# daooshee/ReReVST-Code

Measured on AMD Instinct MI355X. Metric: stylized frames/sec at 512x512, 1 style, higher is better.
Workload: dtype f32

## Files before the change

### include/rerevst_hip.h

```cpp
#ifndef REREVST_HIP_H
#define REREVST_HIP_H

#include <stddef.h>
#include <stdint.h>

#ifdef __cplusplus
extern "C" {
#endif

typedef struct rrv_ctx* rrv_handle;

enum {
    RRV_OK = 0,
    RRV_E_ARG = -1,
    RRV_E_HIP = -2,
    RRV_E_WEIGHTS = -3,
    RRV_E_STATE = -4,
    RRV_E_NOMEM = -5,
    RRV_E_DEBUG = -6,
    RRV_E_COMM = -7
};

#define RRV_STATE_FLOATS 17536
#define RRV_MAX_STYLES 8
// ... 96 lines not shown
#define RRV_TF_ON_STREAM 4
int rrv_transfer_image_device(rrv_handle h, const void* d_in, rrv_image_desc in, int B, int H, int W,
                              void* d_out, rrv_image_desc out, int flags, void* hip_stream);

#define RRV_TF_WEIGHTS_DEVICE (1 << 3)
int rrv_transfer_image_blend_device(rrv_handle h, const void* d_in, rrv_image_desc in, int B, int H, int W,
                                    const float* style_weight, int n_styles,
                                    void* d_out, rrv_image_desc out, int flags, void* hip_stream);
int rrv_transfer_blend_batch(rrv_handle h, const uint8_t* frames_bgr, int B, int H, int W,
                             const float* style_weight, int n_styles, int pad_crop, float* out_bgr),
    rrv_transfer_blend_batch_u8(rrv_handle h, const uint8_t* frames_bgr, int B, int H, int W,
                                const float* style_weight, int n_styles, int pad_crop, uint8_t* out_bgr);

int rrv_transfer_image_mask_device(rrv_handle h, const void* d_in, rrv_image_desc in, int B, int H, int W,
                                   const float* d_mask, int n_styles, int mask_images,
                                   void* d_out, rrv_image_desc out, int flags, void* hip_stream);
int rrv_transfer_mask_batch(rrv_handle h, const uint8_t* frames_bgr, int B, int H, int W,
                            const float* mask, int n_styles, int mask_images, int pad_crop, float* out_bgr),
    rrv_transfer_mask_batch_u8(rrv_handle h, const uint8_t* frames_bgr, int B, int H, int W,
                               const float* mask, int n_styles, int mask_images, int pad_crop, uint8_t* out_bgr);

int rrv_prepare_style_image_device(rrv_handle h, const void* d_style, rrv_image_desc in, int Hs, int Ws, int style_id, void* hip_stream);
int rrv_add_image_device(rrv_handle h, const void* d_frame, rrv_image_desc in, int H, int W, void* hip_stream);

int rrv_get_preclamp(rrv_handle h, float* out, int H, int W);
int rrv_get_preclamp_image(rrv_handle h, float* out, int H, int W, int b);

int rrv_sync(rrv_handle h);

int rrv_set_pipeline(rrv_handle h, int n_slots);

int rrv_set_grid_share(rrv_handle h, int share);

int rrv_set_host_io(rrv_handle h, int mode);

int rrv_debug_copy_tensor(rrv_handle h, int slot, int index, int H, int W, float* host, size_t cap, size_t* floats);

int rrv_debug_copy_tensor_ex(rrv_handle h, int slot, int index, int image, int H, int W, float* host, size_t cap, size_t* floats,
                             int* layout, int* channels);

#define RRV_DBG_STATE_SET 0
#define RRV_DBG_STYLE_PRED 1
int rrv_debug_copy_state(rrv_handle h, int what, int slot, int image, float* out, int n);

int rrv_set_caller_stream(rrv_handle h, void* hip_stream, int enable);

int rrv_host_alloc(size_t bytes, void** out);
int rrv_host_free(void* p);
int rrv_host_register(void* p, size_t bytes);
int rrv_host_unregister(void* p);

int rrv_set_debug(rrv_handle h, int level);
int rrv_debug_selftest(rrv_handle h);
int rrv_debug_fail_alloc(rrv_handle h, int nth);

int rrv_profile_begin(rrv_handle h);
int rrv_profile_end(rrv_handle h);
int rrv_profile_count(rrv_handle h);
int rrv_profile_entry(rrv_handle h, int i, const char** name, float* ms, double* flops, double* bytes,
                      double* flops_executed);

#ifdef __cplusplus
}
#endif
#endif
```

### rerevst-code_amd/_lib.py

```python
import ctypes as C
import os

HERE = os.path.dirname(os.path.abspath(__file__))
LIB_PATH = os.environ.get("RRV_LIB_PATH") or os.path.join(HERE, "librerevst_hip.so")
STATE_FLOATS = 17536
MAX_STYLES = 8

_lib = None


class ImageDesc(C.Structure):
    _fields_ = [("dtype", C.c_int), ("layout", C.c_int), ("space", C.c_int)]


DT_U8, DT_F32 = 0, 1
LAY_HWC_BGR, LAY_CHW_RGB = 0, 1
SP_PIXEL, SP_UNIT, SP_NORM = 0, 1, 2
TF_PAD_CROP, TF_FRAME_MODE, TF_ON_STREAM, TF_WEIGHTS_DEVICE = 1, 2, 4, 8
DBG_STATE_SET, DBG_STYLE_PRED = 0, 1

SYMBOLS = {
    "rrv_create": (C.c_int, [C.c_int, C.POINTER(C.c_void_p)]),
    "rrv_destroy": (C.c_int, [C.c_void_p]),
    "rrv_last_error": (C.c_char_p, [C.c_void_p]),
# ... 13 lines not shown
    "rrv_broadcast_state": (C.c_int, [C.c_void_p, C.c_void_p, C.c_int, C.c_int, C.c_int]),
    "rrv_transfer": (C.c_int, [C.c_void_p, C.c_void_p, C.c_int, C.c_int, C.c_void_p]),
    "rrv_transfer_async": (C.c_int, [C.c_void_p, C.c_void_p, C.c_int, C.c_int, C.c_void_p, C.POINTER(C.c_long)]),
    "rrv_transfer_wait": (C.c_int, [C.c_void_p, C.c_long]),
    "rrv_transfer_device": (C.c_int, [C.c_void_p, C.c_void_p, C.c_int, C.c_int, C.c_void_p]),
    "rrv_transfer_batch_device": (C.c_int, [C.c_void_p, C.c_void_p, C.c_int, C.c_int, C.c_int, C.c_void_p]),
    "rrv_transfer_blend_device": (C.c_int, [C.c_void_p, C.c_void_p, C.c_int, C.c_int, C.POINTER(C.c_float), C.c_int, C.c_void_p]),
    "rrv_transfer_batch": (C.c_int, [C.c_void_p, C.c_void_p, C.c_int, C.c_int, C.c_int, C.c_void_p]),
    "rrv_transfer_blend": (C.c_int, [C.c_void_p, C.c_void_p, C.c_int, C.c_int, C.POINTER(C.c_float), C.c_int, C.c_void_p]),
    "rrv_transfer_frames_device": (C.c_int, [C.c_void_p, C.c_void_p, C.c_int, C.c_int, C.c_int, C.c_void_p]),
    "rrv_transfer_frames": (C.c_int, [C.c_void_p, C.c_void_p, C.c_int, C.c_int, C.c_int, C.c_void_p]),
    "rrv_generate_content_features": (C.c_int, [C.c_void_p, C.c_void_p, C.c_int, C.c_int, C.POINTER(C.c_int)]),
    "rrv_generate_content_features_batch": (C.c_int, [C.c_void_p, C.c_void_p, C.c_int, C.c_int, C.c_int, C.POINTER(C.c_int)]),
    "rrv_add_patch": (C.c_int, [C.c_void_p, C.c_int]),
    "rrv_transfer_features": (C.c_int, [C.c_void_p, C.c_int, C.POINTER(C.c_float), C.c_int, C.c_void_p]),
    "rrv_transfer_features_batch": (C.c_int, [C.c_void_p, C.POINTER(C.c_int), C.POINTER(C.c_float), C.c_int, C.c_int, C.c_void_p]),
    "rrv_release_features": (C.c_int, [C.c_void_p]),
    "rrv_set_multistyle_group": (C.c_int, [C.c_void_p, C.c_int]),
    "rrv_set_f43": (C.c_int, [C.c_void_p, C.c_int]),
    "rrv_set_feature_cache_cap": (C.c_int, [C.c_void_p, C.c_size_t]),
    "rrv_feature_cache_info": (C.c_int, [C.c_void_p, C.POINTER(C.c_int), C.POINTER(C.c_int), C.POINTER(C.c_size_t)]),
    "rrv_transfer_frame_mode": (C.c_int, [C.c_void_p, C.c_void_p, C.c_int, C.c_int, C.c_void_p]),
    "rrv_transfer_frame_mode_batch_device": (C.c_int, [C.c_void_p, C.c_void_p, C.c_int, C.c_int, C.c_int, C.c_void_p]),
    "rrv_transfer_frame_mode_batch": (C.c_int, [C.c_void_p, C.c_void_p, C.c_int, C.c_int, C.c_int, C.c_void_p]),
    "rrv_transfer_frame_mode_frames_device": (C.c_int, [C.c_void_p, C.c_void_p, C.c_int, C.c_int, C.c_int, C.c_void_p]),
    "rrv_transfer_frame_mode_frames": (C.c_int, [C.c_void_p, C.c_void_p, C.c_int, C.c_int, C.c_int, C.c_void_p]),
    "rrv_transfer_image_device": (C.c_int, [C.c_void_p, C.c_void_p, ImageDesc, C.c_int, C.c_int, C.c_int, C.c_void_p, ImageDesc,
                                            C.c_int, C.c_void_p]),
    "rrv_transfer_image_blend_device": (C.c_int, [C.c_void_p, C.c_void_p, ImageDesc, C.c_int, C.c_int, C.c_int, C.c_void_p, C.c_int,
                                                  C.c_void_p, ImageDesc, C.c_int, C.c_void_p]),
    "rrv_transfer_blend_batch": (C.c_int, [C.c_void_p, C.c_void_p, C.c_int, C.c_int, C.c_int, C.POINTER(C.c_float), C.c_int, C.c_int, C.c_void_p]),
    "rrv_transfer_image_mask_device": (C.c_int, [C.c_void_p, C.c_void_p, ImageDesc, C.c_int, C.c_int, C.c_int, C.c_void_p, C.c_int, C.c_int,
                                                 C.c_void_p, ImageDesc, C.c_int, C.c_void_p]),
    "rrv_transfer_mask_batch": (C.c_int, [C.c_void_p, C.c_void_p, C.c_int, C.c_int, C.c_int, C.POINTER(C.c_float), C.c_int, C.c_int, C.c_int, C.c_void_p]),
    "rrv_prepare_style_image_device": (C.c_int, [C.c_void_p, C.c_void_p, ImageDesc, C.c_int, C.c_int, C.c_int, C.c_void_p]),
    "rrv_add_image_device": (C.c_int, [C.c_void_p, C.c_void_p, ImageDesc, C.c_int, C.c_int, C.c_void_p]),
    "rrv_get_preclamp": (C.c_int, [C.c_void_p, C.c_void_p, C.c_int, C.c_int]),
    "rrv_get_preclamp_image": (C.c_int, [C.c_void_p, C.c_void_p, C.c_int, C.c_int, C.c_int]),
    "rrv_sync": (C.c_int, [C.c_void_p]),
    "rrv_set_pipeline": (C.c_int, [C.c_void_p, C.c_int]),
    "rrv_set_host_io": (C.c_int, [C.c_void_p, C.c_int]),
    "rrv_debug_copy_tensor": (C.c_int, [C.c_void_p, C.c_int, C.c_int, C.c_int, C.c_int, C.c_void_p, C.c_size_t, C.POINTER(C.c_size_t)]),
    "rrv_debug_copy_tensor_ex": (C.c_int, [C.c_void_p, C.c_int, C.c_int, C.c_int, C.c_int, C.c_int, C.c_void_p, C.c_size_t,
                                           C.POINTER(C.c_size_t), C.POINTER(C.c_int), C.POINTER(C.c_int)]),
    "rrv_debug_copy_state": (C.c_int, [C.c_void_p, C.c_int, C.c_int, C.c_int, C.c_void_p, C.c_int]),
    "rrv_set_grid_share": (C.c_int, [C.c_void_p, C.c_int]),
    "rrv_set_caller_stream": (C.c_int, [C.c_void_p, C.c_void_p, C.c_int]),
    "rrv_host_alloc": (C.c_int, [C.c_size_t, C.POINTER(C.c_void_p)]),
    "rrv_host_free": (C.c_int, [C.c_void_p]),
    "rrv_host_register": (C.c_int, [C.c_void_p, C.c_size_t]),
    "rrv_host_unregister": (C.c_int, [C.c_void_p]),
    "rrv_set_debug": (C.c_int, [C.c_void_p, C.c_int]),
    "rrv_debug_selftest": (C.c_int, [C.c_void_p]),
    "rrv_debug_fail_alloc": (C.c_int, [C.c_void_p, C.c_int]),
    "rrv_profile_begin": (C.c_int, [C.c_void_p]),
    "rrv_profile_end": (C.c_int, [C.c_void_p]),
    "rrv_profile_count": (C.c_int, [C.c_void_p]),
    "rrv_profile_entry": (C.c_int, [C.c_void_p, C.c_int, C.POINTER(C.c_char_p), C.POINTER(C.c_float),
                                    C.POINTER(C.c_double), C.POINTER(C.c_double), C.POINTER(C.c_double)]),
}

U8_TWINS = ("rrv_transfer", "rrv_transfer_async", "rrv_transfer_batch", "rrv_transfer_frames", "rrv_transfer_device",
            "rrv_transfer_batch_device", "rrv_transfer_frames_device", "rrv_transfer_blend", "rrv_transfer_blend_device",
            "rrv_transfer_features", "rrv_transfer_features_batch", "rrv_transfer_frame_mode", "rrv_transfer_frame_mode_batch",
            "rrv_transfer_frame_mode_batch_device", "rrv_transfer_frame_mode_frames", "rrv_transfer_frame_mode_frames_device",
            "rrv_transfer_blend_batch", "rrv_transfer_mask_batch")
SYMBOLS.update({name + "_u8": SYMBOLS[name] for name in U8_TWINS})


def _share_torch_hip_runtime():
    if os.environ.get("RRV_SYSTEM_HIP") == "1":
        return
    try:
        import importlib.util
        spec = importlib.util.find_spec("torch")
        if spec and spec.submodule_search_locations:
            libdir = os.path.join(list(spec.submodule_search_locations)[0], "lib")
            cand = os.path.join(libdir, "libamdhip64.so")
            if os.path.exists(cand):
                C.CDLL(cand, mode=C.RTLD_GLOBAL)
            rccl = os.path.join(libdir, "librccl.so")
            if os.path.exists(rccl):
                os.environ.setdefault("RRV_RCCL_PATH", rccl)
    except Exception:
        pass


def load():
    global _lib
    if _lib is not None:
        return _lib
    if not os.path.exists(LIB_PATH):
        raise OSError("%s not found: build it with `python __graft_entry__.py build` "
                      "(hipcc --offload-arch=gfx950); there is no CPU fallback" % LIB_PATH)
    _share_torch_hip_runtime()
    lib = C.CDLL(LIB_PATH)
    for name, (res, args) in SYMBOLS.items():
        fn = getattr(lib, name)
        fn.restype, fn.argtypes = res, args
    _lib = lib
    return lib
```

### rerevst-code_amd/csrc/conv_ups5.h

```cpp
#pragma once

struct Ups5Tab {
    static constexpr int G2[5][3] = {{2, 0, 0}, {1, 1, 1}, {-1, -1, 1}, {-1, 1, 1}, {0, 0, 2}};
    static constexpr int BT4[4][4] = {{1, 0, -1, 0}, {0, 1, 1, 0}, {0, -1, 1, 0}, {0, -1, 0, 1}};
    static constexpr int AT[4][5] = {{1, 1, 0, -1, 0}, {0, 1, 1, 0, 0}, {0, 1, 0, 1, 0}, {0, 1, -1, 0, 1}};
    static constexpr int DS[5] = {0, 1, 2, 2, 3};
};
template <int T, int R>
constexpr int ups5_coef(int k) { return T == 0 ? Ups5Tab::BT4[R][k] : Ups5Tab::AT[R][k]; }
template <int T, int R, int N>
__device__ __forceinline__ f32x4 ups5_comb(const f32x4 (&x)[N]) {
    constexpr int F = [] { for (int k = 0; k < N; ++k) if (ups5_coef<T, R>(k) == 1) return k; return -1; }();
    static_assert(F >= 0, "every row has a +1 coefficient");
    f32x4 r = x[F];
    static_for([&](auto kc) {
        constexpr int k = decltype(kc)::value;
        constexpr int c = ups5_coef<T, R>(k);
        static_assert(c == 0 || c == 1 || c == -1, "0 / +-1 coefficients");
        if constexpr (k != F && c == 1) r = e4add(r, x[k]);
        else if constexpr (c == -1) r = f4sub(r, x[k]);
    }, std::make_integer_sequence<int, N>{});
    return r;
}

struct Ups5Geo {
    static constexpr int NT = 256, NB = 2;
    static constexpr int NPOS = 29;
    static constexpr int NUB = 26;
    static constexpr int NPIECE = 16;
    static constexpr int HALO = 18, HALF = 18 * 9;
    static constexpr int PIECES = HALO * HALO * 4;
    static constexpr int RAW_IT = (PIECES + NT - 1) / NT;
    static constexpr int RAW_BYTES = RAW_IT * NT * 16;
    static constexpr int U_BYTES = NUB * 32 * 16 * 4;
    static constexpr int U_IT = U_BYTES / 16 / NT;
    static_assert(U_IT * NT * 16 == U_BYTES, "U image is a whole number of LDS-DMA rounds");
    static constexpr int SMEM = 2 * RAW_BYTES + 2 * U_BYTES + WINO_PAR_BYTES;
    static_assert(SMEM <= 160 * 1024, "LDS");
    static constexpr int OCC = 1;
    static constexpr int vidx(int i) { return i < 25 ? Ups5Tab::DS[i % 5] * 4 + Ups5Tab::DS[i / 5] : (i == 25 ? 5 : i == 26 ? 9 : i == 27 ? 6 : 10); }
    static constexpr int issued(int j) { return (j + 2 < NUB ? 2 : 0) + (j < NPIECE ? 1 : 0); }
    static constexpr int younger(int i) {
        return i == 0 ? 2 + issued(0) : i == 1 ? issued(0) + issued(1) : (i - 2 < NPIECE ? 1 : 0) + issued(i - 1) + issued(i);
    }
    static constexpr int col_iter(int dx) { return 4 * dx + 6; }
    static constexpr int row_iter(int r) { return col_iter(3) + 1 + r; }
};
static_assert(Ups5Geo::row_iter(3) < Ups5Geo::NPOS, "next chunk transformed inside the MFMA loop");

template <int EPI, int PERIMG>
__device__ __forceinline__ void conv_ups5_body(const ConvP& p) {
    static_assert(!(EPI & (E_POOL | E_RES | E_RES_UPS | E_NORM2)), "conv1 epilogues only: bias, activation, saved-stat normalise");
    using G = Ups5Geo;
    constexpr int RAW_BYTES = G::RAW_BYTES, U_BYTES = G::U_BYTES, NT = G::NT, NB = G::NB, NPOS = G::NPOS, NUB = G::NUB;
    extern __shared__ __attribute__((aligned(16))) char smem[];
    const int tid = threadIdx.x;
    const int wave = __builtin_amdgcn_readfirstlane(tid >> 6);
    const int lane = tid & 63, t = lane & 15, q = lane >> 4;
    const int tr = t >> 3, tc = t & 7;
    const int tg = wave;
    const int nchunks = p.Cin >> 4;
    const int n_ntiles = p.Cout >> 5;

    struct Item { int tx, ty, b, nt; };
    Item cur, nxt, dlt;
    {
        const int GD = gridDim.x, w = blockIdx.x;
        int pix, dpix;
        if (p.xcd_slabs) {
            const int PT = (GD >> 3) / n_ntiles;
            pix = (w & 7) * PT + (w >> 3) / n_ntiles; dpix = 8 * PT;
            cur.nt = (w >> 3) % n_ntiles; dlt.nt = 0;
        } else {
            cur.nt = w % n_ntiles; pix = w / n_ntiles;
            dlt.nt = GD % n_ntiles; dpix = GD / n_ntiles;
        }
        cur.tx = pix % p.tiles_x; cur.ty = (pix / p.tiles_x) % p.tiles_y; cur.b = pix / (p.tiles_x * p.tiles_y);
        dlt.tx = dpix % p.tiles_x; dlt.ty = (dpix / p.tiles_x) % p.tiles_y; dlt.b = dpix / (p.tiles_x * p.tiles_y);
    }
    auto advance = [&](const Item& a) {
        Item r = a;
        r.nt += dlt.nt;
        int carry = 0;
        if (r.nt >= n_ntiles) { r.nt -= n_ntiles; carry = 1; }
        r.tx += dlt.tx + carry;
        if (r.tx >= p.tiles_x) { r.tx -= p.tiles_x; r.ty += 1; }
        r.ty += dlt.ty;
        if (r.ty >= p.tiles_y) { r.ty -= p.tiles_y; r.b += 1; }
        r.b += dlt.b;
        return r;
    };
    auto in_of = [&](const Item& a) {
        return p.in + (size_t)a.b * (size_t)(p.Hi + 2) * (p.Wi + 2) * p.Cin + (size_t)(((a.ty + p.ty0) * 16) * (p.Wi + 2) + (a.tx + p.tx0) * 16) * p.Cin;
    };
    auto w_of = [&](const Item& a) { return p.wpk + (size_t)a.nt * nchunks * (NUB * 32 * 16); };
    int asrc[G::RAW_IT];
#pragma unroll
    for (int it = 0; it < G::RAW_IT; ++it) {
        const int e = it * NT + tid;
        int P = e >> 2;
        const int qq = e & 3;
        if (P >= G::HALO * G::HALO) P = 0;
        const int hf = P >= G::HALF, rem = P - hf * G::HALF;
        const int hy = rem / 9, hx = 2 * (rem - hy * 9) + hf;
        asrc[it] = ((hy * (p.Wi + 2) + hx) * p.Cin + 4 * (qq ^ ((hx >> 1) & 3))) * 4;
    }
    const int raw_last_num = ((G::RAW_IT - 1) * NT + wave * 64 < G::PIECES) ? 0x7fffffff : 0;
    bool have = cur.b < p.B, have_nxt = false;
    const float* in_t = in_of(cur);
    const float* w_t = w_of(cur);
    const float* in_n = in_t;
    const float* w_n = w_t;
    auto stage_u = [&](int chunk) {
        char* udst = smem + 2 * RAW_BYTES + (chunk & 1) * U_BYTES;
#pragma unroll
        for (int it = 0; it < G::U_IT; ++it) bufld16(w_t, udst + (it * NT + wave * 64) * 16, tid * 16, chunk * U_BYTES + it * NT * 16);
    };
    auto stage_raw = [&](int chunk) {
        char* rdst = smem + (chunk & 1) * RAW_BYTES;
#pragma unroll
        for (int it = 0; it < G::RAW_IT; ++it)
            if (it * NT + wave * 64 < G::PIECES) bufld16(in_t, rdst + (it * NT + wave * 64) * 16, asrc[it], chunk * 64);
    };
    char* const par = smem + 2 * RAW_BYTES + 2 * U_BYTES;
    auto stage_params = [&](int ntile, int img) {
        if (wave < 2) {
            const int e = tid;
            const int row = e >> 3, col = (e & 7) * 4;
            const float* src = p.bias;
            const int pb = PERIMG ? img * p.par_bstride : 0;
            int off = ntile * 32 + col;
            if (row >= 1 && row <= 4) { src = (EPI & E_NORM1) ? p.n1 : p.bias; off = (EPI & E_NORM1) ? ntile * 32 + col + pb + (row - 1) * p.Cout : off; }
            if (row > 4) { src = p.bias; off = ntile * 32; }
            glds16(src + off, par + wave * 1024);
        }
    };

    const unsigned lds0 = (unsigned)(size_t)(__attribute__((address_space(3))) char*)smem;
    unsigned offD[4];
#pragma unroll
    for (int dx = 0; dx < 4; ++dx) {
        const int hy = 4 * tg + 2 * tr, hx = 2 * tc + dx;
        const int P = (hx & 1) * G::HALF + hy * 9 + (hx >> 1);
        offD[dx] = lds0 + P * 64 + ((q ^ ((hx >> 1) & 3)) << 4);
    }
    const unsigned offU = lds0 + 2 * RAW_BYTES + t * 64 + ((q ^ ((0 - (t >> 2)) & 3)) << 4);
    const unsigned offU1 = offU + U_BYTES;

    f32x4 acc[NPOS][NB];
    f32x4 va[16], vb[16];
    auto pass = [](f32x4& x0, f32x4& x1, f32x4& x2, f32x4& x3) {
        const f32x4 a[4] = {x0, x1, x2, x3};
        x0 = ups5_comb<0, 0>(a); x1 = ups5_comb<0, 1>(a); x2 = ups5_comb<0, 2>(a); x3 = ups5_comb<0, 3>(a);
    };
    auto col_pass = [&](f32x4 (&d)[16], int dx) { pass(d[dx * 4 + 0], d[dx * 4 + 1], d[dx * 4 + 2], d[dx * 4 + 3]); };
    auto row_pass = [&](f32x4 (&d)[16], int r) { pass(d[0 * 4 + r], d[1 * 4 + r], d[2 * 4 + r], d[3 * 4 + r]); };

    auto chunk_body = [&](int c, auto par_c, auto first_c, f32x4 (&vcur)[16], f32x4 (&vnext)[16]) {
        constexpr int PAR = decltype(par_c)::value;
        constexpr bool FIRST = decltype(first_c)::value;
        const bool own_u = c + 1 < nchunks, own_r = c + 2 < nchunks;
        const rsrc_t rs_u = make_rsrc(own_u ? w_t : w_n);
        const rsrc_t rs_r = make_rsrc(own_r ? in_t : in_n);
        const rsrc_t rs_rl = make_rsrc(own_r ? in_t : in_n, raw_last_num);
        const int usoff = own_u ? (c + 1) * U_BYTES : 0;
        const int rsoff = (own_r ? c + 2 : c + 2 - nchunks) * 64;
        char* const udst = smem + 2 * RAW_BYTES + (1 - PAR) * U_BYTES;
        char* const rdst = smem + PAR * RAW_BYTES;
        const unsigned ub = PAR ? offU1 : offU;
        constexpr int RB = (1 - PAR) * RAW_BYTES;
        f32x4 u[4][NB];
        f32x4 (&d)[16] = vnext;
        u[0][0] = lds_rd128<0>(ub);
        u[0][1] = lds_rd128<1024>(ub);
        u[1][0] = lds_rd128<2048>(ub);
        u[1][1] = lds_rd128<2048 + 1024>(ub);
        static_for([&](auto ic) {
            constexpr int i = decltype(ic)::value;
            if constexpr (i + 2 < NUB) {
                u[(i + 2) & 3][0] = lds_rd128<(i + 2) * 2048>(ub);
                u[(i + 2) & 3][1] = lds_rd128<(i + 2) * 2048 + 1024>(ub);
            }
            if constexpr (i < 16) d[i] = lds_rd128<RB + (i & 3) * 576>(offD[i >> 2]);
            constexpr int US = (i < NUB ? i : NUB - 1) & 3;
            if constexpr (i < NUB) {
                constexpr int cdx = (i - 6) / 4;
                if constexpr (i >= 6 && (i - 6) % 4 == 0 && cdx < 4) {
                    static_assert(G::col_iter(cdx) == i, "column release schedule");
                    asm volatile("s_waitcnt lgkmcnt(%6)" : "+v"(d[cdx * 4 + 0]), "+v"(d[cdx * 4 + 1]), "+v"(d[cdx * 4 + 2]), "+v"(d[cdx * 4 + 3]),
                                 "+v"(u[US][0]), "+v"(u[US][1]) : "i"(G::younger(i)));
                } else {
                    lds_release2<G::younger(i)>(u[US][0], u[US][1]);
                }
            }
            __builtin_amdgcn_sched_barrier(0);
            if constexpr (i < G::U_IT) bufld16_rs(rs_u, udst + (i * NT + wave * 64) * 16, tid * 16, usoff + i * NT * 16);
            if constexpr (i < G::RAW_IT) bufld16_rs(i == G::RAW_IT - 1 ? rs_rl : rs_r, rdst + (i * NT + wave * 64) * 16, asrc[i], rsoff);
            const f32x4 vv = vcur[G::vidx(i)];
#pragma unroll
            for (int s = 0; s < 4; ++s)
#pragma unroll
                for (int nb = 0; nb < NB; ++nb)
                    acc[i][nb] = __builtin_amdgcn_mfma_f32_16x16x4f32(u[US][nb][s], vv[s], (FIRST && s == 0) ? f32x4{0.f, 0.f, 0.f, 0.f} : acc[i][nb], 0, 0, 0);
            static_for([&](auto xc) {
                constexpr int k = decltype(xc)::value;
                if constexpr (G::col_iter(k) == i) col_pass(d, k);
                if constexpr (G::row_iter(k) == i) row_pass(d, k);
            }, std::make_integer_sequence<int, 4>{});
        }, std::make_integer_sequence<int, NPOS>{});
    };

    int par_ntile = -1, par_img = -1;
    if (have) {
        stage_raw(0);
        stage_u(0);
        stage_raw(1);
        stage_params(cur.nt, cur.b);
        par_ntile = cur.nt; par_img = cur.b;
        __syncthreads();
#pragma unroll
        for (int k = 0; k < 16; ++k) va[k] = *(const f32x4*)(smem + (offD[k >> 2] - lds0) + (k & 3) * 576);
#pragma unroll
        for (int dx = 0; dx < 4; ++dx) col_pass(va, dx);
#pragma unroll
        for (int r = 0; r < 4; ++r) row_pass(va, r);
        __syncthreads();
    }
    while (have) {
        const int e_y0 = (cur.ty + p.ty0) * 32, e_x0 = (cur.tx + p.tx0) * 32, e_b = cur.b, e_ntile = cur.nt;
        nxt = advance(cur);
        have_nxt = nxt.b < p.B;
        in_n = have_nxt ? in_of(nxt) : in_t;
        w_n = have_nxt ? w_of(nxt) : w_t;
        if (par_ntile != e_ntile || (PERIMG && par_img != e_b)) {
            __syncthreads();
            stage_params(e_ntile, e_b);
            par_ntile = e_ntile; par_img = e_b;
        }
        chunk_body(0, std::integral_constant<int, 0>{}, std::true_type{}, va, vb);
        __syncthreads();
        chunk_body(1, std::integral_constant<int, 1>{}, std::false_type{}, vb, va);
        __syncthreads();
        for (int c = 2; c < nchunks; c += 2) {
            chunk_body(c, std::integral_constant<int, 0>{}, std::false_type{}, va, vb);
            __syncthreads();
            chunk_body(c + 1, std::integral_constant<int, 1>{}, std::false_type{}, vb, va);
            __syncthreads();
        }
        cur = nxt; have = have_nxt; in_t = in_n; w_t = w_n;

        float* out_b = p.out + (size_t)e_b * (size_t)(p.H + 2) * (p.W + 2 + (p.out_p8 ? 6 : 0)) * p.Cout;
        const int yb = e_y0 + 8 * tg + 4 * tr, xb = e_x0 + 4 * tc;
        {
            const int ly0 = yb >> 1, lx0 = xb >> 1;
            float* sc_b = p.sc_out + (size_t)e_b * (size_t)(p.Hi + 2) * (p.Wi + 2) * p.Cout;
#pragma unroll
            for (int nb = 0; nb < NB; ++nb) {
                const f32x4 s0 = f4sub(acc[25][nb], acc[27][nb]), s1 = e4add(acc[25][nb], acc[27][nb]);
                const f32x4 t0 = f4sub(acc[26][nb], acc[28][nb]), t1 = e4add(acc[26][nb], acc[28][nb]);
                const f32x4 sc[2][2] = {{f4sub(s0, t0), e4add(s0, t0)}, {f4sub(s1, t1), e4add(s1, t1)}};
#pragma unroll
                for (int a = 0; a < 2; ++a)
#pragma unroll
                    for (int b = 0; b < 2; ++b) {
                        const int ly = ly0 + a, lx = lx0 + b;
                        if (ly < p.Hi && lx < p.Wi)
                            *(f32x4*)(sc_b + ((size_t)(ly + 1) * (p.Wi + 2) + lx + 1) * p.Cout + e_ntile * 32 + nb * 16 + 4 * q) = sc[a][b];
                    }
            }
        }
#pragma unroll
        for (int nb = 0; nb < NB; ++nb) {
            const int co = e_ntile * 32 + nb * 16 + 4 * q;
            f32x4 T[5][4];
#pragma unroll
            for (int r = 0; r < 5; ++r) {
                const f32x4 m[5] = {acc[r * 5 + 0][nb], acc[r * 5 + 1][nb], acc[r * 5 + 2][nb], acc[r * 5 + 3][nb], acc[r * 5 + 4][nb]};
                T[r][0] = ups5_comb<1, 0>(m); T[r][1] = ups5_comb<1, 1>(m); T[r][2] = ups5_comb<1, 2>(m); T[r][3] = ups5_comb<1, 3>(m);
            }
            f32x4 Y[4][4];
#pragma unroll
            for (int j = 0; j < 4; ++j) {
                const f32x4 tj[5] = {T[0][j], T[1][j], T[2][j], T[3][j], T[4][j]};
                Y[0][j] = ups5_comb<1, 0>(tj); Y[1][j] = ups5_comb<1, 1>(tj); Y[2][j] = ups5_comb<1, 2>(tj); Y[3][j] = ups5_comb<1, 3>(tj);
            }
            const char* pl = par + (nb * 16 + 4 * q) * 4;
            const f32x4 bias = *(const f32x4*)(pl);
            f32x4 m1, r1, lo1, hi1;
            if (EPI & E_NORM1) {
                m1 = *(const f32x4*)(pl + 128); r1 = *(const f32x4*)(pl + 256);
                lo1 = *(const f32x4*)(pl + 384); hi1 = *(const f32x4*)(pl + 512);
            }
#pragma unroll
            for (int i = 0; i < 4; ++i)
#pragma unroll
                for (int j = 0; j < 4; ++j) {
                    const int y = yb + i, x = xb + j;
                    f32x4 o = e4add(Y[i][j], bias);
                    if (EPI & E_RELU) o = f4relu(o);
                    if (EPI & E_LRELU) o = f4lrelu(o);
                    if (EPI & E_NORM1) o = f4norm_clamp(o, m1, r1, lo1, hi1);
                    if (y < p.H && x < p.W) {
                        if (p.out_p8) *(f32x4*)(out_b + (size_t)(co >> 3) * ((size_t)(p.H + 2) * (p.W + 8) * 8) + ((size_t)(y + 1) * (p.W + 8) + x + 4) * 8 + (co & 7)) = o;
                        else *(f32x4*)(out_b + ((size_t)(y + 1) * (p.W + 2) + x + 1) * p.Cout + co) = o;
                    }
                }
        }
    }
    asm volatile("s_waitcnt vmcnt(0)" ::: "memory");
}

__global__ void pack_ups5_k(const float* __restrict__ w, const float* __restrict__ wsc, float* __restrict__ dst, int Cout, int Cin) {
    constexpr int CH = 16, NUB = Ups5Geo::NUB;
    const size_t total = (size_t)Cout * Cin * NUB;
    for (size_t i = blockIdx.x * (size_t)blockDim.x + threadIdx.x; i < total; i += (size_t)gridDim.x * blockDim.x) {
        size_t r = i;
        const int cl = (int)(r % CH); r /= CH;
        const int j = r & 31; r >>= 5;
        const int pos = (int)(r % NUB); r /= NUB;
        const int nchunks = Cin / CH;
        const int chunk = r % nchunks; r /= nchunks;
        const int n_tile = (int)r;
        const int e = cl & 3, qs = cl >> 2;
        const int qq = qs ^ ((0 - (j >> 2)) & 3);
        const int co = n_tile * 32 + j, ci = chunk * CH + qq * 4 + e;
        if (pos == 25) { dst[i] = wsc[(size_t)co * Cin + ci] * 0.25f; continue; }
        const float* g = w + ((size_t)co * Cin + ci) * 9;
        auto G5 = [](int row, double g0, double g1, double g2) {
            return 0.5 * (Ups5Tab::G2[row][0] * g0 + Ups5Tab::G2[row][1] * g1 + Ups5Tab::G2[row][2] * g2);
        };
        const int pr = pos / 5, pc = pos % 5;
        double rowv[3];
#pragma unroll
        for (int kx = 0; kx < 3; ++kx) rowv[kx] = G5(pr, g[0 * 3 + kx], g[1 * 3 + kx], g[2 * 3 + kx]);
        dst[i] = (float)G5(pc, rowv[0], rowv[1], rowv[2]);
    }
}
```

### rerevst-code_amd/csrc/rerevst_hip.hip

```cpp
#include <hip/hip_runtime.h>
#include <dlfcn.h>
#include <stddef.h>
#include <stdint.h>
#include <string.h>
#include <algorithm>
#include <cmath>
#include <thread>
#include <stdio.h>
#include <map>
#include <condition_variable>
#include <mutex>
#include <string>
#include <vector>

#include "../../include/rerevst_hip.h"
#include "conv_mfma.h"
#include "conv_wino.h"
#include "conv_wino_split.h"
#include "conv_f43.h"
#include "conv_thin.h"
#include "prep_kernels.h"
#include "mask_kernels.h"

namespace {
// ... 1553 lines not shown
    if (const char* e = getenv("RRV_DEBUG")) h->debug = atoi(e) < 0 ? 0 : (atoi(e) > 2 ? 2 : atoi(e));
    *out = h;
    return RRV_OK;
}

static void free_plans(rrv_handle h) {
    for (auto& pair : h->enc_frame) for (EncPlan& e : pair) enc_free(e);
    enc_free(h->enc_add); enc_free(h->enc_style);
    for (auto& pair : h->dec) for (DecPlan& d : pair) dec_free(h, d);
    prep_free(h);
}

int rrv_set_debug(rrv_handle h, int level) {
    if (!h || level < 0 || level > 2) return RRV_E_ARG;
    HIPCHK(hipSetDevice(h->dev));
    RCHK(sync_all(h));
    free_plans(h);
    h->debug = level;
    return RRV_OK;
}

int rrv_debug_fail_alloc(rrv_handle h, int nth) {
    if (!h || nth < 0) return RRV_E_ARG;
    h->fail_alloc_in = nth;
    return RRV_OK;
}

__global__ void dbg_poke_k(float* p, long off) { p[off] = 1.0f; }
int rrv_debug_selftest(rrv_handle h) {
    if (!h) return RRV_E_ARG;
    HIPCHK(hipSetDevice(h->dev));
    RCHK(sync_all(h));
    const int saved = h->debug;
    h->debug = 2;
    Tens t;
    int rc = talloc(h, &t, 2, 8, 8, 64);
    if (rc == RRV_OK) rc = debug_verify(h, "selftest (clean)");
    int caught = 0;
    if (rc == RRV_OK) {
        hipLaunchKernelGGL(dbg_poke_k, dim3(1), dim3(1), 0, h->stream, t.p, (long)t.img_floats() + 5);
        if (debug_verify(h, "selftest (ring)") == RRV_E_DEBUG) ++caught;
        HIPCHK(hipMemsetAsync(t.p + t.img_floats(), 0, 64 * sizeof(float), h->stream));
        hipLaunchKernelGGL(dbg_poke_k, dim3(1), dim3(1), 0, h->stream, t.p, -3L);
        if (debug_verify(h, "selftest (guard)") == RRV_E_DEBUG) ++caught;
    }
    tfree(&t);
    h->debug = saved;
    if (rc != RRV_OK) return rc;
    if (caught != 2) return fail(h, RRV_E_DEBUG, "debug selftest: a deliberate out-of-bounds store was not detected");
    h->err.clear();
    return RRV_OK;
}

int rrv_destroy(rrv_handle h) {
    if (!h) return RRV_E_ARG;
    (void)hipSetDevice(h->dev);
    (void)hipDeviceSynchronize();
    for (auto& kv : h->conv) {
        if (kv.second.raw) (void)hipFree(kv.second.raw);
        if (kv.second.pk) (void)hipFree(kv.second.pk);
        if (kv.second.pk_ups) (void)hipFree(kv.second.pk_ups);
        if (kv.second.pk_ups_sc) (void)hipFree(kv.second.pk_ups_sc);
        if (kv.second.pk_wino) (void)hipFree(kv.second.pk_wino);
        if (kv.second.pk_f43) (void)hipFree(kv.second.pk_f43);
        if (kv.second.bias && kv.second.bias != h->zero_bias) (void)hipFree(kv.second.bias);
    }
    if (h->zero_bias) (void)hipFree(h->zero_bias);
    for (int f = 0; f < 3; ++f) {
        const ConvW &fd = h->sets[0].fold_down[f], &fu = h->sets[0].fold_up[f];
        for (float* q : {fd.raw, fd.bias, fd.pk_wino, fu.raw, fu.pk_wino}) if (q) (void)hipFree(q);
    }
    if (h->sets[0].active) (void)hipFree(h->sets[0].active);
    for (int i = 0; i < 6; ++i) { if (h->fc_w[i]) (void)hipFree(h->fc_w[i]); if (h->fc_b[i]) (void)hipFree(h->fc_b[i]); }
    if (h->fold_tmp) (void)hipFree(h->fold_tmp);
    for (float* p : h->patches) (void)hipFree(p);
    for (auto& f : h->features) if (f.owned) { if (f.p) (void)hipFree(f.p); if (f.u8) (void)hipFree(f.u8); }
    for (void* b : h->feat_blocks) (void)hipFree(b);
    free_plans(h);
    for (StyleState& s : h->styles) { if (s.blob) (void)hipFree(s.blob); if (s.smean) (void)hipFree(s.smean); tfree(&s.map); }
    if (h->d_u8) (void)hipFree(h->d_u8);
    if (h->d_outf) (void)hipFree(h->d_outf);
    if (h->pend_u8) (void)hipFree(h->pend_u8);
    for (auto& bw : h->blend_w) {
        if (bw.dev) (void)hipFree(bw.dev);
        if (bw.pin) (void)hipHostFree(bw.pin);
        for (hipEvent_t e : bw.ev) if (e) (void)hipEventDestroy(e);
    }
    if (h->stat_part) (void)hipFree(h->stat_part);
    for (float* q : {h->first_w[0], h->first_w[1], h->first_b[0], h->first_b[1], h->first_wg}) if (q) (void)hipFree(q);
    for (auto& st : h->hstage) {
        stage_free(st.pin, true);
        stage_free(st.dev, false);
        if (st.mask) (void)hipFree(st.mask);
        if (st.mask_pin) (void)hipHostFree(st.mask_pin);
        for (hipEvent_t e : {st.in_done, st.k_done, st.out_done}) if (e) (void)hipEventDestroy(e);
    }
    if (h->copy_in) (void)hipStreamDestroy(h->copy_in);
    if (h->copy_out) (void)hipStreamDestroy(h->copy_out);
    for (ProfEntry& e : h->prof) { (void)hipEventDestroy(e.e0); (void)hipEventDestroy(e.e1); }
    for (int i = 0; i < RRV_MAX_SLOTS; ++i) { (void)hipStreamDestroy(h->streams[i]); if (h->slot_ev[i]) (void)hipEventDestroy(h->slot_ev[i]); }
    delete h;
    return RRV_OK;
}

const char* rrv_last_error(rrv_handle h) { return h ? h->err.c_str() : "null handle"; }

// ... 1540 lines not shown
```

### rerevst-code_amd/framework.py

```python
import collections
import ctypes as C

import numpy as np

from . import _lib
from .weights import weight_table, load_checkpoint


class RRVError(RuntimeError):
    pass


def pinned_empty(shape, dtype=np.float32):
    import weakref
    lib = _lib.load()
    dt = np.dtype(dtype)
    n = int(np.prod(shape)) * dt.itemsize
    ptr = C.c_void_p()
    if lib.rrv_host_alloc(max(n, 1), C.byref(ptr)) != 0:
        raise MemoryError("rrv_host_alloc(%d) failed" % n)
    buf = (C.c_char * max(n, 1)).from_address(ptr.value)
    weakref.finalize(buf, lib.rrv_host_free, ptr)
    return np.frombuffer(buf, dtype=dt, count=int(np.prod(shape))).reshape(shape)

# ... 218 lines not shown
        self._h = C.c_void_p()
        rc = self._lib.rrv_create(self.device, C.byref(self._h))
        if rc != 0:
            self._h = None
            raise RRVError("rrv_create(device=%d) failed with %d (no HIP device?)" % (self.device, rc))
        weights = checkpoint if isinstance(checkpoint, dict) else load_checkpoint(checkpoint)
        for key, shape in weight_table().items():
            if key not in weights:
                raise KeyError("missing weight %s" % key)
            w = np.ascontiguousarray(weights[key], dtype=np.float32)
            if tuple(w.shape) != tuple(shape):
                raise ValueError("weight %s has shape %s, expected %s" % (key, w.shape, shape))
            shp = (C.c_int64 * w.ndim)(*w.shape)
            self._chk(self._lib.rrv_load_weight(self._h, key.encode(), w.ctypes.data_as(C.c_void_p), shp, w.ndim))
        self._chk(self._lib.rrv_finalize_weights(self._h))

    def _chk(self, rc):
        if rc != 0:
            msg = self._lib.rrv_last_error(self._h)
            err = RRVError("librerevst_hip error %d: %s" % (rc, msg.decode() if msg else "?"))
            err.code = rc
            raise err

    def close(self):
        if getattr(self, "_h", None):
            self._lib.rrv_destroy(self._h)
            self._h = None
        self._open = {}

    def __del__(self):
        try:
            self.close()
        except Exception:
            pass

    def _global_only(self, what):
        if not self.use_Global:
            raise RRVError("%s() belongs to Sequence-Level Global Feature Sharing (use_Global=True)" % what)

    def add(self, patch):
        self._global_only("add")
        a = _u8_image(patch, "patch")
        self._chk(self._lib.rrv_add(self._h, a.ctypes.data_as(C.c_void_p), a.shape[0], a.shape[1]))

    def compute(self):
        self._global_only("compute")
        self._chk(self._lib.rrv_compute(self._h))

    def set_debug(self, level):
        self._chk(self._lib.rrv_set_debug(self._h, int(level)))

    def debug_selftest(self):
        self._chk(self._lib.rrv_debug_selftest(self._h))

    def debug_fail_alloc(self, nth):
        self._chk(self._lib.rrv_debug_fail_alloc(self._h, int(nth)))

    def set_workspace_cap(self, nbytes):
        self._chk(self._lib.rrv_set_workspace_cap(self._h, int(nbytes)))

    def last_compute_info(self):
        g, n, b = C.c_int(), C.c_int(), C.c_size_t()
        self._chk(self._lib.rrv_last_compute_info(self._h, C.byref(g), C.byref(n), C.byref(b)))
        return g.value, n.value, b.value

    def clean(self):
        self._global_only("clean")
        self._chk(self._lib.rrv_clean(self._h))

    def prepare_style(self, style):
        styles = style if isinstance(style, (list, tuple)) else [style]
        for sid, s in enumerate(styles):
            a = _u8_image(s, "style")
            self._chk(self._lib.rrv_prepare_style(self._h, a.ctypes.data_as(C.c_void_p), a.shape[0], a.shape[1], sid))

    def _device_image(self, x, space, layout):
        import torch
        a = tensor_io_args(x, self.device, space=space, layout=layout)
        return a, C.c_void_p(torch.cuda.current_stream(x.device).cuda_stream)

    def prepare_style_tensor(self, style, *, space="pixel", layout="nchw"):
        styles = style if isinstance(style, (list, tuple)) else [style]
        for sid, s in enumerate(styles):
            a, stream = self._device_image(s, space, layout)
            if a.batched:
                raise ValueError("a style is one image: [3,H,W] or [H,W,3], got shape %s" % (tuple(s.shape),))
            self._chk(self._lib.rrv_prepare_style_image_device(self._h, C.c_void_p(a.x.data_ptr()), a.in_desc, a.H, a.W, sid, stream))

    def add_tensor(self, x, *, space="pixel", layout="nchw"):
        self._global_only("add")
        a, stream = self._device_image(x, space, layout)
        xb = a.x if a.batched else a.x.unsqueeze(0)
        for b in range(a.B):
            self._chk(self._lib.rrv_add_image_device(self._h, C.c_void_p(xb[b].data_ptr()), a.in_desc, a.H, a.W, stream))

    def transfer(self, frame, style_weight=None, dtype=np.float32):
        a = _u8_image(frame, "frame")
        H, W = a.shape[:2]
        out, u8 = _output((H // 8 * 8, W // 8 * 8, 3), dtype, None)
        if not self.use_Global:
            fn = self._lib.rrv_transfer_frame_mode_u8 if u8 else self._lib.rrv_transfer_frame_mode
            self._chk(fn(self._h, a.ctypes.data_as(C.c_void_p), H, W, out.ctypes.data_as(C.c_void_p)))
            return out
        if style_weight is None:
            fn = self._lib.rrv_transfer_u8 if u8 else self._lib.rrv_transfer
            rc = fn(self._h, a.__array_interface__["data"][0], H, W, out.__array_interface__["data"][0])
# ... 285 lines not shown
```

Before: 852.6.

## Spread ups5 conv prefetch requests across MFMA loop and double-buffer epilogue params

Spreads the global-to-LDS buffer loads for the next chunk's raw input and transformed weights evenly across the MFMA iterations (SPAN=25), where before they were issued in a burst at the first iterations. Epilogue parameters (bias and normalisation stats) are double-buffered in LDS and staged for the next tile during the current one, which removes an extra __syncthreads before each parameter restage. Adds compile-time ablation switches and a debug entry point for testing the conv kernel in isolation. The risk is different instruction scheduling and register pressure inside the hot loop.

```diff
diff --git a/include/rerevst_hip.h b/include/rerevst_hip.h
--- a/include/rerevst_hip.h
+++ b/include/rerevst_hip.h
@@ -172,6 +172,8 @@
 
 int rrv_set_debug(rrv_handle h, int level);
 int rrv_debug_selftest(rrv_handle h);
+int rrv_debug_conv_ups5(rrv_handle h, const float* in_ring, int B, int Hi, int Wi, int Cin, int Cout, const float* w, const float* wsc,
+                        const float* bias, const float* n1, int per_image, int out_p8, int grid_wgs, float* out, float* sc_out);
 int rrv_debug_fail_alloc(rrv_handle h, int nth);
 
 int rrv_profile_begin(rrv_handle h);
diff --git a/rerevst-code_amd/_lib.py b/rerevst-code_amd/_lib.py
--- a/rerevst-code_amd/_lib.py
+++ b/rerevst-code_amd/_lib.py
@@ -89,6 +89,8 @@
     "rrv_host_unregister": (C.c_int, [C.c_void_p]),
     "rrv_set_debug": (C.c_int, [C.c_void_p, C.c_int]),
     "rrv_debug_selftest": (C.c_int, [C.c_void_p]),
+    "rrv_debug_conv_ups5": (C.c_int, [C.c_void_p, C.c_void_p, C.c_int, C.c_int, C.c_int, C.c_int, C.c_int, C.c_void_p, C.c_void_p,
+                                      C.c_void_p, C.c_void_p, C.c_int, C.c_int, C.c_int, C.c_void_p, C.c_void_p]),
     "rrv_debug_fail_alloc": (C.c_int, [C.c_void_p, C.c_int]),
     "rrv_profile_begin": (C.c_int, [C.c_void_p]),
     "rrv_profile_end": (C.c_int, [C.c_void_p]),
diff --git a/rerevst-code_amd/csrc/conv_ups5.h b/rerevst-code_amd/csrc/conv_ups5.h
--- a/rerevst-code_amd/csrc/conv_ups5.h
+++ b/rerevst-code_amd/csrc/conv_ups5.h
@@ -1,4 +1,14 @@
 #pragma once
+
+#ifndef UPS5_ABL
+#define UPS5_ABL 0
+#endif
+#ifndef UPS5_SPAN
+#define UPS5_SPAN 25
+#endif
+#ifndef UPS5_PARDB
+#define UPS5_PARDB 1
+#endif
 
 struct Ups5Tab {
     static constexpr int G2[5][3] = {{2, 0, 0}, {1, 1, 1}, {-1, -1, 1}, {-1, 1, 1}, {0, 0, 2}};
@@ -45,13 +55,20 @@
     }
     static constexpr int col_iter(int dx) { return 4 * dx + 6; }
     static constexpr int row_iter(int r) { return col_iter(3) + 1 + r; }
+    static constexpr int NREQ = U_IT + RAW_IT, SPAN = UPS5_SPAN;
+    static constexpr bool req_raw(int n) { return n % 3 == 0 && n / 3 < RAW_IT; }
+    static constexpr int req_idx(int n) { int k = 0; for (int m = 0; m < n; ++m) k += req_raw(m) == req_raw(n); return k; }
+    static constexpr int req_iter(int n) { return SPAN ? n * SPAN / NREQ : req_idx(n); }
 };
+static_assert(Ups5Geo::SPAN >= 0 && Ups5Geo::SPAN <= Ups5Geo::NPOS && Ups5Geo::req_raw(15) && !Ups5Geo::req_raw(18) && Ups5Geo::req_idx(18) == Ups5Geo::U_IT - 1, "every request inside the MFMA loop");
 static_assert(Ups5Geo::row_iter(3) < Ups5Geo::NPOS, "next chunk transformed inside the MFMA loop");
 
 template <int EPI, int PERIMG>
 __device__ __forceinline__ void conv_ups5_body(const ConvP& p) {
     static_assert(!(EPI & (E_POOL | E_RES | E_RES_UPS | E_NORM2)), "conv1 epilogues only: bias, activation, saved-stat normalise");
     using G = Ups5Geo;
+    constexpr int ABL = UPS5_ABL, PARDB = UPS5_PARDB;
+    static_assert(!PARDB || 2 * 1024 <= WINO_PAR_BYTES, "two parameter images");
     constexpr int RAW_BYTES = G::RAW_BYTES, U_BYTES = G::U_BYTES, NT = G::NT, NB = G::NB, NPOS = G::NPOS, NUB = G::NUB;
     extern __shared__ __attribute__((aligned(16))) char smem[];
     const int tid = threadIdx.x;
@@ -123,8 +140,8 @@
             if (it * NT + wave * 64 < G::PIECES) bufld16(in_t, rdst + (it * NT + wave * 64) * 16, asrc[it], chunk * 64);
     };
     char* const par = smem + 2 * RAW_BYTES + 2 * U_BYTES;
-    auto stage_params = [&](int ntile, int img) {
-        if (wave < 2) {
+    auto stage_params = [&](int ntile, int img, int slot) {
+        if (wave < (PARDB ? 1 : 2)) {
             const int e = tid;
             const int row = e >> 3, col = (e & 7) * 4;
             const float* src = p.bias;
@@ -132,7 +149,7 @@
             int off = ntile * 32 + col;
             if (row >= 1 && row <= 4) { src = (EPI & E_NORM1) ? p.n1 : p.bias; off = (EPI & E_NORM1) ? ntile * 32 + col + pb + (row - 1) * p.Cout : off; }
             if (row > 4) { src = p.bias; off = ntile * 32; }
-            glds16(src + off, par + wave * 1024);
+            glds16(src + off, par + (PARDB ? slot : wave) * 1024);
         }
     };
 
@@ -194,28 +211,41 @@
                 }
             }
             __builtin_amdgcn_sched_barrier(0);
-            if constexpr (i < G::U_IT) bufld16_rs(rs_u, udst + (i * NT + wave * 64) * 16, tid * 16, usoff + i * NT * 16);
-            if constexpr (i < G::RAW_IT) bufld16_rs(i == G::RAW_IT - 1 ? rs_rl : rs_r, rdst + (i * NT + wave * 64) * 16, asrc[i], rsoff);
+            if constexpr (!(ABL & 1) && G::SPAN == 0) {
+                if constexpr (i < G::U_IT) bufld16_rs(rs_u, udst + (i * NT + wave * 64) * 16, tid * 16, usoff + i * NT * 16);
+                if constexpr (i < G::RAW_IT) bufld16_rs(i == G::RAW_IT - 1 ? rs_rl : rs_r, rdst + (i * NT + wave * 64) * 16, asrc[i], rsoff);
+            } else if constexpr (!(ABL & 1)) {
+                static_for([&](auto nc) {
+                    constexpr int n = decltype(nc)::value, k = G::req_idx(n);
+                    if constexpr (G::req_iter(n) == i) {
+                        if constexpr (G::req_raw(n)) bufld16_rs(k == G::RAW_IT - 1 ? rs_rl : rs_r, rdst + (k * NT + wave * 64) * 16, asrc[k], rsoff);
+                        else bufld16_rs(rs_u, udst + (k * NT + wave * 64) * 16, tid * 16, usoff + k * NT * 16);
+                    }
+                }, std::make_integer_sequence<int, G::NREQ>{});
+            }
             const f32x4 vv = vcur[G::vidx(i)];
 #pragma unroll
             for (int s = 0; s < 4; ++s)
 #pragma unroll
                 for (int nb = 0; nb < NB; ++nb)
                     acc[i][nb] = __builtin_amdgcn_mfma_f32_16x16x4f32(u[US][nb][s], vv[s], (FIRST && s == 0) ? f32x4{0.f, 0.f, 0.f, 0.f} : acc[i][nb], 0, 0, 0);
-            static_for([&](auto xc) {
-                constexpr int k = decltype(xc)::value;
-                if constexpr (G::col_iter(k) == i) col_pass(d, k);
-                if constexpr (G::row_iter(k) == i) row_pass(d, k);
-            }, std::make_integer_sequence<int, 4>{});
+            if constexpr (!(ABL & 8)) {
+                static_for([&](auto xc) {
+                    constexpr int k = decltype(xc)::value;
+                    if constexpr (G::col_iter(k) == i) col_pass(d, k);
+                    if constexpr (G::row_iter(k) == i) row_pass(d, k);
+                }, std::make_integer_sequence<int, 4>{});
+            }
         }, std::make_integer_sequence<int, NPOS>{});
     };
-
-    int par_ntile = -1, par_img = -1;
+    auto barrier_chunk = [&]() { if constexpr (!(ABL & 2)) __syncthreads(); };
+
+    int par_ntile = -1, par_img = -1, par_slot = 0, par_flip = 0;
     if (have) {
         stage_raw(0);
         stage_u(0);
         stage_raw(1);
-        stage_params(cur.nt, cur.b);
+        stage_params(cur.nt, cur.b, 0);
         par_ntile = cur.nt; par_img = cur.b;
         __syncthreads();
 #pragma unroll
@@ -232,22 +262,43 @@
         have_nxt = nxt.b < p.B;
         in_n = have_nxt ? in_of(nxt) : in_t;
         w_n = have_nxt ? w_of(nxt) : w_t;
-        if (par_ntile != e_ntile || (PERIMG && par_img != e_b)) {
-            __syncthreads();
-            stage_params(e_ntile, e_b);
-            par_ntile = e_ntile; par_img = e_b;
+        if constexpr (!PARDB) {
+            if (par_ntile != e_ntile || (PERIMG && par_img != e_b)) {
+                __syncthreads();
+                stage_params(e_ntile, e_b, 0);
+                par_ntile = e_ntile; par_img = e_b;
+            }
         }
         chunk_body(0, std::integral_constant<int, 0>{}, std::true_type{}, va, vb);
-        __syncthreads();
+        barrier_chunk();
+        if constexpr (PARDB) {
+            if (have_nxt && (par_ntile != nxt.nt || (PERIMG && par_img != nxt.b))) {
+                par_slot ^= 1;
+                stage_params(nxt.nt, nxt.b, par_slot);
+                par_ntile = nxt.nt; par_img = nxt.b;
+                par_flip = 1;
+            }
+        }
         chunk_body(1, std::integral_constant<int, 1>{}, std::false_type{}, vb, va);
-        __syncthreads();
+        barrier_chunk();
         for (int c = 2; c < nchunks; c += 2) {
             chunk_body(c, std::integral_constant<int, 0>{}, std::false_type{}, va, vb);
-            __syncthreads();
+            barrier_chunk();
             chunk_body(c + 1, std::integral_constant<int, 1>{}, std::false_type{}, vb, va);
-            __syncthreads();
+            barrier_chunk();
         }
         cur = nxt; have = have_nxt; in_t = in_n; w_t = w_n;
+        const char* const par_e = par + (PARDB ? (par_slot ^ par_flip) * 1024 : 0);
+        par_flip = 0;
+        if constexpr ((ABL & 32) != 0) {
+            f32x4 sacc = acc[0][0];
+#pragma unroll
+            for (int i = 0; i < NPOS; ++i)
+#pragma unroll
+                for (int nb = 0; nb < NB; ++nb) if (i || nb) sacc += acc[i][nb];
+            if (sacc[0] + sacc[1] + sacc[2] + sacc[3] == 123.456f) p.out[tid] = sacc[0];
+            continue;
+        }
 
         float* out_b = p.out + (size_t)e_b * (size_t)(p.H + 2) * (p.W + 2 + (p.out_p8 ? 6 : 0)) * p.Cout;
         const int yb = e_y0 + 8 * tg + 4 * tr, xb = e_x0 + 4 * tc;
@@ -264,8 +315,11 @@
 #pragma unroll
                     for (int b = 0; b < 2; ++b) {
                         const int ly = ly0 + a, lx = lx0 + b;
-                        if (ly < p.Hi && lx < p.Wi)
-                            *(f32x4*)(sc_b + ((size_t)(ly + 1) * (p.Wi + 2) + lx + 1) * p.Cout + e_ntile * 32 + nb * 16 + 4 * q) = sc[a][b];
+                        if (ly < p.Hi && lx < p.Wi) {
+                            float* const dst = sc_b + ((size_t)(ly + 1) * (p.Wi + 2) + lx + 1) * p.Cout + e_ntile * 32 + nb * 16 + 4 * q;
+                            if constexpr ((ABL & 4) != 0) { if (sc[a][b][0] == 123.456f) *dst = sc[a][b][0]; }
+                            else *(f32x4*)dst = sc[a][b];
+                        }
                     }
             }
         }
@@ -284,7 +338,7 @@
                 const f32x4 tj[5] = {T[0][j], T[1][j], T[2][j], T[3][j], T[4][j]};
                 Y[0][j] = ups5_comb<1, 0>(tj); Y[1][j] = ups5_comb<1, 1>(tj); Y[2][j] = ups5_comb<1, 2>(tj); Y[3][j] = ups5_comb<1, 3>(tj);
             }
-            const char* pl = par + (nb * 16 + 4 * q) * 4;
+            const char* pl = par_e + (nb * 16 + 4 * q) * 4;
             const f32x4 bias = *(const f32x4*)(pl);
             f32x4 m1, r1, lo1, hi1;
             if (EPI & E_NORM1) {
@@ -301,7 +355,8 @@
                     if (EPI & E_LRELU) o = f4lrelu(o);
                     if (EPI & E_NORM1) o = f4norm_clamp(o, m1, r1, lo1, hi1);
                     if (y < p.H && x < p.W) {
-                        if (p.out_p8) *(f32x4*)(out_b + (size_t)(co >> 3) * ((size_t)(p.H + 2) * (p.W + 8) * 8) + ((size_t)(y + 1) * (p.W + 8) + x + 4) * 8 + (co & 7)) = o;
+                        if constexpr ((ABL & 4) != 0) { if (o[0] == 123.456f) out_b[co] = o[0]; }
+                        else if (p.out_p8) *(f32x4*)(out_b + (size_t)(co >> 3) * ((size_t)(p.H + 2) * (p.W + 8) * 8) + ((size_t)(y + 1) * (p.W + 8) + x + 4) * 8 + (co & 7)) = o;
                         else *(f32x4*)(out_b + ((size_t)(y + 1) * (p.W + 2) + x + 1) * p.Cout + co) = o;
                     }
                 }
diff --git a/rerevst-code_amd/csrc/rerevst_hip.hip b/rerevst-code_amd/csrc/rerevst_hip.hip
--- a/rerevst-code_amd/csrc/rerevst_hip.hip
+++ b/rerevst-code_amd/csrc/rerevst_hip.hip
@@ -1629,6 +1629,54 @@
     return RRV_OK;
 }
 
+int rrv_debug_conv_ups5(rrv_handle h, const float* in_ring, int B, int Hi, int Wi, int Cin, int Cout, const float* w, const float* wsc,
+                        const float* bias, const float* n1, int per_image, int out_p8, int grid_wgs, float* out, float* sc_out) {
+    if (!h || !in_ring || !w || !wsc || !bias || !n1 || !out || !sc_out) return RRV_E_ARG;
+    if (B < 1 || Hi < 1 || Wi < 1 || Cin < 64 || (Cin & 31) || Cout < 32 || (Cout & 31) || grid_wgs < 0 || grid_wgs > 4096) return RRV_E_ARG;
+    HIPCHK(hipSetDevice(h->dev));
+    RCHK(sync_all(h));
+    constexpr int EPI = E_LRELU | E_NORM1;
+    const int H = 2 * Hi, W = 2 * Wi, images = per_image ? B : 1;
+    Tens ti, to, ts;
+    ConvW cw, cs;
+    float *dbias = nullptr, *dn1 = nullptr;
+    cw.Cout = cs.Cout = Cout; cw.Cin = cs.Cin = Cin; cw.taps = 9; cs.taps = 1;
+    auto body = [&]() -> int {
+        RCHK(talloc(h, &ti, B, Hi, Wi, Cin));
+        RCHK(out_p8 ? talloc(h, &to, B * (Cout / 8), H, W + 6, 8) : talloc(h, &to, B, H, W, Cout));
+        RCHK(talloc(h, &ts, B, Hi, Wi, Cout));
+        RCHK(dalloc(h, &cw.raw, (size_t)Cout * Cin * 9, false)); RCHK(dalloc(h, &cs.raw, (size_t)Cout * Cin, false));
+        RCHK(dalloc(h, &dbias, Cout, false)); RCHK(dalloc(h, &dn1, (size_t)images * 4 * Cout, false));
+        HIPCHK(hipMemcpyAsync(ti.p, in_ring, (size_t)B * ti.img_floats() * sizeof(float), hipMemcpyHostToDevice, h->stream));
+        HIPCHK(hipMemcpyAsync(cw.raw, w, (size_t)Cout * Cin * 9 * sizeof(float), hipMemcpyHostToDevice, h->stream));
+        HIPCHK(hipMemcpyAsync(cs.raw, wsc, (size_t)Cout * Cin * sizeof(float), hipMemcpyHostToDevice, h->stream));
+        HIPCHK(hipMemcpyAsync(dbias, bias, (size_t)Cout * sizeof(float), hipMemcpyHostToDevice, h->stream));
+        HIPCHK(hipMemcpyAsync(dn1, n1, (size_t)images * 4 * Cout * sizeof(float), hipMemcpyHostToDevice, h->stream));
+        RCHK(pack_ups_sc(h, cw, cs));
+        ConvP p{};
+        p.in = ti.p; p.Hi = Hi; p.Wi = Wi; p.Cin = Cin; p.out = to.p; p.H = H; p.W = W; p.Cout = Cout; p.B = B; p.in_bstride0 = 1;
+        p.wpk = cw.pk_ups_sc; p.bias = dbias; p.n1 = dn1; p.sc_out = ts.p; p.out_p8 = out_p8 ? 1 : 0;
+        p.par_bstride = per_image ? 4 * Cout : 0;
+        p.tiles_x = (W + 31) / 32; p.tiles_y = (H + 31) / 32;
+        const unsigned slabs = (unsigned)(Cout / 32), items = (unsigned)(p.tiles_x * p.tiles_y * B) * slabs, resident = resident_wgs(h, Ups5Geo::OCC);
+        const dim3 grid(grid_wgs ? (unsigned)grid_wgs : (items < resident ? items : resident), 1);
+        p.xcd_slabs = (grid.x % 8 == 0 && (grid.x / 8) % slabs == 0) ? 1 : 0;
+        HIPCHK((wino_attr<EPI, UPW_NW, 1, 1, 1>()));
+        if (per_image) wino_launch<EPI, UPW_NW, 1, 1, 1>(p, grid, h->stream);
+        else wino_launch<EPI, UPW_NW, 1, 1, 0>(p, grid, h->stream);
+        HIPCHK(hipGetLastError());
+        HIPCHK(hipMemcpyAsync(out, to.p, (size_t)to.B * to.img_floats() * sizeof(float), hipMemcpyDeviceToHost, h->stream));
+        HIPCHK(hipMemcpyAsync(sc_out, ts.p, (size_t)B * ts.img_floats() * sizeof(float), hipMemcpyDeviceToHost, h->stream));
+        HIPCHK(hipStreamSynchronize(h->stream));
+        return h->debug ? debug_verify(h, "debug_conv_ups5") : RRV_OK;
+    };
+    const int rc = body();
+    (void)hipStreamSynchronize(h->stream);
+    tfree(&ti); tfree(&to); tfree(&ts);
+    for (float* q : {cw.raw, cs.raw, cw.pk_ups_sc, dbias, dn1}) if (q) (void)hipFree(q);
+    return rc;
+}
+
 int rrv_destroy(rrv_handle h) {
     if (!h) return RRV_E_ARG;
     (void)hipSetDevice(h->dev);
diff --git a/rerevst-code_amd/framework.py b/rerevst-code_amd/framework.py
--- a/rerevst-code_amd/framework.py
+++ b/rerevst-code_amd/framework.py
@@ -294,6 +294,20 @@
 
     def debug_selftest(self):
         self._chk(self._lib.rrv_debug_selftest(self._h))
+
+    def debug_conv_ups5(self, x, w, wsc, bias, n1, out_p8=False, grid=0):
+        x = np.ascontiguousarray(x, np.float32)
+        B, Hi, Wi, Cin = x.shape
+        Cout = int(w.shape[0])
+        ring = np.ascontiguousarray(np.pad(x, ((0, 0), (1, 1), (1, 1), (0, 0))))
+        w, wsc, bias, n1 = (np.ascontiguousarray(a, np.float32) for a in (w, wsc, bias, n1))
+        assert w.shape == (Cout, Cin, 3, 3) and wsc.size == Cout * Cin and bias.size == Cout and n1.shape in ((4, Cout), (B, 4, Cout))
+        H, W = 2 * Hi, 2 * Wi
+        out = np.empty((B, (H + 2) * (W + 8) * Cout if out_p8 else (H + 2) * (W + 2) * Cout), np.float32)
+        sc = np.empty((B, (Hi + 2) * (Wi + 2) * Cout), np.float32)
+        self._chk(self._lib.rrv_debug_conv_ups5(self._h, ring.ctypes.data, B, Hi, Wi, Cin, Cout, w.ctypes.data, wsc.ctypes.data, bias.ctypes.data,
+                                                n1.ctypes.data, int(n1.ndim == 3), int(bool(out_p8)), int(grid), out.ctypes.data, sc.ctypes.data))
+        return out, sc
 
     def debug_fail_alloc(self, nth):
         self._chk(self._lib.rrv_debug_fail_alloc(self._h, int(nth)))
```

Measured after the change: 853.5, median of 2. No clear change (+0.1%).
